# FabianPlum/SMILify

Measured on AMD Instinct MI355X. Metric: SMIL fit-iters/sec (LBS+render+loss) per GPU at 1/2/4/8 MI355X, higher is better.
Workload: dtype f32

## Files before the change

smilify_amd/csrc/raster.hip:

```cpp
#include "common.h"

#include "raster_hooks.h"
#include "raster_common.h"
#include "raster_setup.h"
#include "raster_tile.h"
#include "raster_replay.h"

static int device_cus() { return smil_device_limits().cus; }

static long long tile_slots() {
    long long resident = (long long)device_cus() * RESIDENT_PER_CU;
    HOOK_RESIDENT(resident)
    return resident;
}
static int tile_grid(int N, int tiles_x) {
    const long long resident = tile_slots();
    const unsigned long long n_max = (unsigned long long)N * tiles_x * tiles_x;
    const unsigned int slots = (unsigned int)resident;
    unsigned int best = slots / 8u;
    const unsigned long long ends[4] = {slots * 5ull / 64ull, slots * 5ull / 16ull, slots * 5ull / 8ull, n_max};
    for (int k = 0; k < 4; ++k) {
        const unsigned long long n = ends[k] < n_max ? ends[k] : n_max;
        if (n == 0ull || n > 0x7FFFFFFull) { if (n) best = slots; continue; }
        const unsigned int w = deal_working((unsigned int)n, deal_split_log((unsigned int)n, slots), slots);
// ... 18 lines not shown
    a.fzr = q.fzr = w.take<float2>((size_t)N * FT);
    a.gbox = q.gbox = w.take<uint32_t>((size_t)N * (FT / WAVE));
    a.img_bound = q.img_bound = w.take<float>(N);
    a.loss_acc = q.loss_acc = w.take<unsigned long long>(N);
    a.list_cap = q.list_cap = list_cap_of(m, S);
    a.lists = q.lists = w.take<uint2>((size_t)N * q.list_cap);
    ClipTables &c = q.clip;
    c.xv = w.take<float>((size_t)N * CLIP_VX * 3);
    c.xg = w.take<float>((size_t)N * CLIP_VX * 2);
    c.xsrc = w.take<int2>((size_t)N * CLIP_VX);
    c.xcoef = w.take<float2>((size_t)N * CLIP_VX);
    c.xf = w.take<int>((size_t)N * CLIP_FX * 3);
    c.xcount = w.take<uint32_t>(N);
    c.xparent = nullptr;
    a.clip = c;
    w.take<char>(256);
    const size_t grid = (size_t)tile_grid(N, tiles_x);
    a.list_stride = (int)(align256((size_t)FT * sizeof(uint32_t)) / sizeof(uint32_t));
    a.n_cf = (int)(align256((size_t)(FT / DCHUNK + 2) * sizeof(uint32_t)) / sizeof(uint32_t));
    a.slist = w.take<uint2>(grid * a.list_stride);
    a.slist2 = w.take<uint32_t>(grid * a.list_stride);
    a.scfirst = w.take<uint32_t>(grid * a.n_cf);
    a.sxy = w.take<float2>(grid * a.list_stride * 3);
    a.sid = w.take<TriIds>(grid * a.list_stride);
    a.srec = w.take<Rec3>(grid * (REC_CAP + REC_PAD));
    a.crec = w.take<Rec3>(grid * (REC_CAP + REC_PAD));
    return w.used;
}

extern "C" size_t smil_raster_workspace_bytes(const SmilModel *m, int32_t N, int32_t S) {
    SetupArgs q;
    RasterArgs a;
    return (m && N > 0 && S > 0) ? raster_layout(m, N, S, nullptr, q, a) : 0;
}

extern "C" int smil_raster_stats(const SmilModel *m, const void *workspace, void *stream_, uint32_t *out4) {
    SMIL_REQUIRE(m && workspace && out4, "smil_raster_stats: bad argument");
    RasterCounters h;
    SMIL_HIP(hipMemcpyAsync(&h, workspace, sizeof(h), hipMemcpyDeviceToHost, (hipStream_t)stream_));
    SMIL_HIP(hipStreamSynchronize((hipStream_t)stream_));
    unsigned int tiles = 0;
    for (int q = 0; q < N_PARTS; ++q)
        for (int c = 0; c < N_CLASSES; ++c) tiles += h.n_class[q][c];
    out4[0] = h.straddling; out4[1] = tiles; out4[2] = h.unclipped; out4[3] = h.tie_pixels;
    return SMIL_OK;
}

static int check_sizes(const SmilModel *m, int N, int S, const char *who) {
    SMIL_REQUIRE(N > 0 && S > 0 && S <= TILE * 256, "%s: bad sizes N=%d S=%d", who, N, S);
    const int tiles_x = ceil_div(S, TILE);
    SMIL_REQUIRE((double)N * tiles_x * tiles_x < 2147483647.0, "%s: N * tiles exceeds the work-item index range (2^31); launch in slices", who);
    SMIL_REQUIRE(face_rows(m) + 64 < (1 << 24) && (double)list_cap_of(m, S) * sizeof(uint2) < 4294967296.0,
                 "%s: per-workgroup / per-image tables exceed the 24-bit index / 32-bit byte-offset range of at()", who);
    return SMIL_OK;
}

static int launch_setup(SetupArgs &q, int N, hipStream_t stream) {
    SMIL_HIP(hipMemsetAsync(q.ctr, 0, sizeof(RasterCounters), stream));
    const int n_tiles = q.tiles_x * q.tiles_x;
    q.copies = n_tiles * 2 * 12 <= 48 * 1024 ? 2 : 1;
#ifdef SETUP_COPIES
    q.copies = SETUP_COPIES;
#endif
    const size_t setup_lds = n_tiles <= COUNT_TILES_MAX ? (size_t)n_tiles * q.copies * 12 : (size_t)((n_tiles + 31) / 32) * sizeof(uint32_t);
    hipLaunchKernelGGL(k_raster_setup, dim3(N), dim3(SETUP_THREADS), setup_lds, stream, q);
    SMIL_LAUNCH_CHECK();
    return SMIL_OK;
}

static int raster_common(const SmilModel *m, const float *verts_ndc, int N, int S, const SmilRasterSettings *rs, void *workspace,
                         hipStream_t stream, bool grads, SetupArgs &q, RasterArgs &a) {
    SMIL_REQUIRE(m && verts_ndc && rs && workspace, "raster: null argument");
    if (int rc = check_sizes(m, N, S, "raster")) return rc;
    SMIL_REQUIRE(rs->faces_per_pixel > 0 && rs->faces_per_pixel <= SMIL_MAX_FACES_PER_PIXEL,
                 "raster: faces_per_pixel=%d outside 1..%d", rs->faces_per_pixel, SMIL_MAX_FACES_PER_PIXEL);
    SMIL_REQUIRE(rs->sigma > 0.f && rs->blur_radius >= 0.f, "raster: bad blend settings");
    SMIL_REQUIRE(rs->tie_rule == SMIL_TIE_DEPTH_FACE_ID || rs->tie_rule == SMIL_TIE_REFERENCE_QUEUE, "raster: tie_rule=%d is neither 0 nor 1", rs->tie_rule);
    SMIL_REQUIRE(face_rows(m) <= REC_CAP, "raster: %d faces exceed the %d a single pixel's records may hold", m->F, REC_CAP - CLIP_FX - WAVE);
    static_assert(REC_CAP + REC_PAD < (1 << 24), "at<12-byte>() multiplies 24-bit indices");
    if (grads && rs->clip_depth)
        SMIL_REQUIRE(rs->clip_depth->vertex && rs->clip_depth->dz && rs->clip_depth->range && rs->clip_depth->counter && rs->clip_depth->capacity >= 0 &&
                     rs->image0 >= 0, "raster: incomplete SmilClipDepth");
    raster_layout(m, N, S, (char *)workspace, q, a);
    const int tiles_x = ceil_div(S, TILE);
    if (rs->tie_rule) SMIL_HIP(hipMemsetAsync(a.tie_mask, 0, (size_t)2 * N_PARTS * a.item_cap * sizeof(unsigned long long), stream));
    q.verts_ndc = a.verts_ndc = verts_ndc; q.faces = a.faces = m->faces;
    q.V = a.V = m->V; q.F = a.F = m->F; q.S = a.S = S; q.tiles_x = a.tiles_x = tiles_x;
    q.sqrt_blur = a.sqrt_blur = sqrtf(rs->blur_radius); q.z_clip = rs->z_clip; q.max_valence = m->max_valence;
    q.inv_sigma = a.inv_sigma = 1.0f / rs->sigma;
    q.cd_counter = (grads && rs->clip_depth && rs->image0 == 0) ? rs->clip_depth->counter : nullptr;
    if (int rc = launch_setup(q, N, stream)) return rc;
    a.FT = face_rows(m); a.slots = (unsigned int)tile_slots();
    a.tie_rule = rs->tie_rule; a.image0 = rs->image0;
    a.cd = (grads && rs->clip_depth) ? *rs->clip_depth : SmilClipDepth{nullptr, nullptr, nullptr, nullptr, 0};
    a.N = N; a.K = rs->faces_per_pixel; a.packed = 0;
    a.blur = rs->blur_radius; a.inv_sigma_log2e = (float)(1.4426950408889634 / (double)rs->sigma);
    HOOK_HOST_LAUNCH_SETUP(a, stream)
    a.sil = nullptr; a.grad_sil = nullptr; a.target = nullptr; a.target_u8 = nullptr; a.pix_scale = nullptr; a.loss_img = nullptr;
    a.d_ndc = nullptr;
    return SMIL_OK;
}

static size_t colour_setup_layout(const SmilModel *m, int N, int S, char *base, ColourSetup *o, SetupArgs *q) {
    const int tiles_x = ceil_div(S, TILE), FT = face_rows(m);
    const uint32_t item_cap = (uint32_t)ceil_div(N, N_PARTS) * (uint32_t)(tiles_x * tiles_x);
    const uint32_t list_cap = list_cap_of(m, S);
    Workspace w{base};
    uint32_t *tbox = w.take<uint32_t>((size_t)N * FT);
    RasterCounters *c = w.take<RasterCounters>(1);
    uint4 *items = w.take<uint4>((size_t)2 * N_PARTS * item_cap);
    float2 *fzr = w.take<float2>((size_t)N * FT);
    uint32_t *gbox = w.take<uint32_t>((size_t)N * (FT / WAVE));
    uint2 *lists = w.take<uint2>((size_t)N * list_cap);
    ClipTables clip;
    clip.xv = w.take<float>((size_t)N * CLIP_VX * 3);
    clip.xsrc = w.take<int2>((size_t)N * CLIP_VX);
    clip.xcoef = w.take<float2>((size_t)N * CLIP_VX);
    clip.xf = w.take<int>((size_t)N * CLIP_FX * 3);
    clip.xparent = w.take<int>((size_t)N * CLIP_CUTS);
    clip.xg = nullptr; clip.xcount = nullptr;
    if (!base) return w.used;
    o->tbox = tbox; o->gbox = gbox; o->fzr = fzr; o->items = items;
    o->n_class = &c->n_class[0][0]; o->ticket = &c->deal[0].next; o->item_cap = item_cap;
    o->lists = lists; o->list_cap = list_cap;
    o->xv = clip.xv; o->xf = clip.xf; o->xsrc = clip.xsrc; o->xparent = clip.xparent;
    o->FT = FT; o->FP = faces_padded(m->F); o->clip_vx = CLIP_VX; o->clip_fx = CLIP_FX; o->n_parts = N_PARTS; o->n_classes = N_CLASSES;
    *q = SetupArgs{};
    q->clip = clip; q->faces = m->faces; q->tbox = tbox; q->gbox = gbox; q->items = items;
    q->item_cap = item_cap; q->fzr = fzr; q->ctr = c; q->V = m->V; q->F = m->F; q->S = S; q->tiles_x = tiles_x;
    q->sqrt_blur = 0.f; q->inv_sigma = 1.f; q->lists = lists; q->list_cap = list_cap;
    return w.used;
}

size_t smil_colour_setup_bytes(const SmilModel *m, int N, int S) {
    return (m && N > 0 && S > 0) ? colour_setup_layout(m, N, S, nullptr, nullptr, nullptr) : 0;
}

int smil_colour_setup(const SmilModel *m, const float *verts_ndc, int N, int S, float z_clip, void *workspace, hipStream_t stream,
                      ColourSetup *out) {
    if (int rc = check_sizes(m, N, S, "smil_render_colour")) return rc;
    SetupArgs q;
    colour_setup_layout(m, N, S, (char *)workspace, out, &q);
    q.verts_ndc = verts_ndc; q.z_clip = z_clip;
    return launch_setup(q, N, stream);
}

#define PROF_SLOTS 512
static bool g_prof_on = false;
static hipEvent_t g_prof_ev[PROF_SLOTS][2];
static int g_prof_n = 0;
static bool g_prof_init = false;

extern "C" int smil_profile_enable(int32_t on) {
    if (on && !g_prof_init) {
        for (int i = 0; i < PROF_SLOTS; ++i) {
            SMIL_HIP(hipEventCreate(&g_prof_ev[i][0]));
            SMIL_HIP(hipEventCreate(&g_prof_ev[i][1]));
        }
        g_prof_init = true;
    }
    g_prof_on = on != 0;
    g_prof_n = 0;
    return SMIL_OK;
}

extern "C" int smil_profile_read(float *total_ms, int32_t *launches) {
    SMIL_REQUIRE(total_ms && launches, "smil_profile_read: null argument");
    float tot = 0.f;
    const int n = g_prof_n < PROF_SLOTS ? g_prof_n : PROF_SLOTS;
    for (int i = 0; i < n; ++i) {
        SMIL_HIP(hipEventSynchronize(g_prof_ev[i][1]));
        float ms = 0.f;
        SMIL_HIP(hipEventElapsedTime(&ms, g_prof_ev[i][0], g_prof_ev[i][1]));
        tot += ms;
    }
    *total_ms = tot;
    *launches = n;
    g_prof_n = 0;
    return SMIL_OK;
}

#define PROF_BEGIN(stream) \
    const int _slot = (g_prof_on && g_prof_n < PROF_SLOTS) ? g_prof_n++ : -1; \
    if (_slot >= 0) (void)hipEventRecord(g_prof_ev[_slot][0], stream)
#define PROF_END(stream) \
    if (_slot >= 0) (void)hipEventRecord(g_prof_ev[_slot][1], stream)

template <int MODE>
static void launch_tie_replay(const RasterArgs &a, hipStream_t stream) {
    const size_t lds = (size_t)a.FT / 8 + 6 * WAVE * sizeof(uint32_t) + (size_t)TIE_ORD_CAP * sizeof(uint16_t) + TIE_ORD_CAP / 8;
    if (a.tie_rule) hipLaunchKernelGGL((k_raster_tie_replay<MODE>), dim3((unsigned int)device_cus() * 4u * TIE_WAVES_PER_SIMD), dim3(64), lds, stream, a);
}
template <int MODE>
static int launch_raster(const RasterArgs &a, hipStream_t stream) {
    PROF_BEGIN(stream);
    hipLaunchKernelGGL((k_raster_dense<MODE>), dim3(tile_grid(a.N, a.tiles_x)), dim3(64), 0, stream, a);
    PROF_END(stream);
    launch_tie_replay<MODE>(a, stream);
    SMIL_LAUNCH_CHECK();
    return SMIL_OK;
}

extern "C" int smil_silhouette_forward(const SmilModel *m, const float *verts_ndc, int32_t N, int32_t S,
                                       const SmilRasterSettings *rs, float *sil, void *workspace, void *stream_) {
    hipStream_t stream = (hipStream_t)stream_;
    SetupArgs q{};
    RasterArgs a;
    int rc = raster_common(m, verts_ndc, N, S, rs, workspace, stream, false, q, a);
    if (rc) return rc;
    SMIL_REQUIRE(sil, "smil_silhouette_forward: null output");
    SMIL_HIP(hipMemsetAsync(sil, 0, (size_t)N * S * S * sizeof(float), stream));
    a.sil = sil;
    return launch_raster<MODE_FWD>(a, stream);
// ... 45 lines not shown
```

smilify_amd/csrc/raster_common.h:

```cpp
#pragma once

#define DCHUNK 32
#define FREC 28
#define FSTR 28
#define K_EPS 1e-8f
#define ALPHA_GRAD_EPS 1e-12f
#ifndef SEL_BITS
#define SEL_BITS 5
#endif
#ifndef SEL1_BITS
#define SEL1_BITS 6
#endif
#define SAT8 160u
#ifndef DGROUP
#define DGROUP 4
#endif
#ifndef KGROUP
#define KGROUP 4
#endif
#ifndef SELR
#define SELR 6
#endif
#ifndef LIST_LDS_ROWS
#define LIST_LDS_ROWS 8
// ... 68 lines not shown
struct RasterArgs {
    const float *verts_ndc;
    const int *faces;
    const uint32_t *tbox;
    const uint32_t *gbox;
    const uint4 *items;
    uint32_t item_cap;
    const float2 *fzr;
    RasterCounters *ctr;
    int N, V, F, S, tiles_x, K;
    int FT;
    ClipTables clip;
    float blur, sqrt_blur, inv_sigma, inv_sigma_log2e;
    float *sil;
    const float *grad_sil;
    const float *target;
    const uint8_t *target_u8;
    const float *pix_scale;
    const float *img_bound;
    int packed;
    float *loss_img;
    unsigned long long *loss_acc;
    float *d_ndc;
    const uint2 *lists;
    uint32_t list_cap;
    uint2 *slist;
    uint32_t *slist2;
    uint32_t *scfirst;
    float2 *sxy;
    TriIds *sid;
    Rec3 *srec;
    Rec3 *crec;
    int list_stride, n_cf;
    unsigned int slots;
    SmilClipDepth cd;
    int image0;
    int tie_rule;
    unsigned long long *tie_mask;
    HOOK_ARGS_FIELDS
};

__device__ __forceinline__ float tile_centre(int t, int S) { return pix_to_ndc(S - 1 - (t * TILE + TILE / 2), S); }

__device__ __forceinline__ float edge_fn(float px, float py, float ax, float ay, float bx, float by) {
    return (px - ax) * (by - ay) - (py - ay) * (bx - ax);
}

__device__ __forceinline__ float image_fx_scale(float img_bound, float pix_scale, float inv_sigma) {
    const float bound = img_bound * fabsf(pix_scale) * sqrtf(inv_sigma);
    return (bound > 0.f && bound < 3.0e38f) ? exp2f(fminf(29.0f - floorf(log2f(bound)), 100.0f)) : 0.f;
}

template <typename T>
__device__ __forceinline__ uint32_t byte_offset(uint32_t i) {
    if (sizeof(T) == 12) {
        uint32_t r;
        asm("v_mul_u32_u24 %0, %1, 12" : "=v"(r) : "v"(i));
        return r;
    }
    return i * (uint32_t)sizeof(T);
}
template <typename T>
__device__ __forceinline__ T &at(T *base, uint32_t i) {
    i = HOOK_WRAP_IDX(i);
    return *reinterpret_cast<T *>(reinterpret_cast<char *>(base) + byte_offset<T>(i));
}
template <typename T>
__device__ __forceinline__ const T &at(const T *base, uint32_t i) {
    i = HOOK_WRAP_IDX(i);
    return *reinterpret_cast<const T *>(reinterpret_cast<const char *>(base) + byte_offset<T>(i));
}

__device__ __forceinline__ int wave_scan_add(int x) {
#define SCAN_STEP(ctrl, rows) { x += __builtin_amdgcn_update_dpp(0, x, ctrl, rows, 0xF, false); }
    SCAN_STEP(0x111, 0xF) SCAN_STEP(0x112, 0xF) SCAN_STEP(0x114, 0xF) SCAN_STEP(0x118, 0xF)
    SCAN_STEP(0x142, 0xA) SCAN_STEP(0x143, 0xC)
#undef SCAN_STEP
    return x;
}

#ifndef SETUP_THREADS
#define SETUP_THREADS 1024
#endif
#ifndef LIST_CAP_PER_FACE
#define LIST_CAP_PER_FACE 8
#endif
struct SetupArgs {
    ClipTables clip;
    const float *verts_ndc; const int *faces;
    uint32_t *tbox, *gbox; uint4 *items; uint32_t item_cap; float2 *fzr;
    RasterCounters *ctr;
    int V, F, S, tiles_x; float sqrt_blur, z_clip;
    float *d_ndc_zero; const float *loss_src; float *loss_dst; unsigned long long *loss_acc; float *img_bound; int max_valence;
    float *dndc_scale; const float *pix_scale; float inv_sigma; int packed;
    uint2 *lists;
    uint32_t list_cap;
    uint32_t *cd_counter;
    int copies;
};

struct alignas(16) FaceRec {
    float A0, A1, B0, B1;
    float C0, C1, A2, B2;
    float C2, z0, z1, z2;
    float x0c, x1c, y0c, y1c;
    float e01x, e02x, e01y, e02y;
    float rl01, rl02, e12x, e12y;
    float rl12;
    int i0, i1, i2;
};
static_assert(sizeof(FaceRec) == FREC * sizeof(float), "FaceRec layout");

typedef float f32x2 __attribute__((ext_vector_type(2)));
__device__ __forceinline__ f32x2 splat2(float x) { return (f32x2){x, x}; }
__device__ __forceinline__ f32x2 clamp01(f32x2 v) {
    return __builtin_elementwise_min(__builtin_elementwise_max(v, splat2(0.f)), splat2(1.f));
}
__device__ __forceinline__ float vmax_raw(float a, float b) {
    float r;
    asm("v_max_f32 %0, %1, %2" : "=v"(r) : "v"(a), "v"(b));
    return r;
}

struct FaceRows { float4 r0, r1, r2, r3, r4, r5, r6; };
struct PairEval2 {
    f32x2 w0, w1, w2;
    f32x2 sd;
    bool cand0, cand1, inside0, inside1;
    uint32_t ebits0, ebits1;
};
__device__ __forceinline__ f32x2 pk_fma(f32x2 a, f32x2 b, f32x2 c) { return __builtin_elementwise_fma(a, b, c); }
__device__ __forceinline__ f32x2 pk_mul_clamp_lo(f32x2 v, f32x2 s2) {
    f32x2 r;
    asm("v_pk_mul_f32 %0, %1, %2 op_sel_hi:[1,0] clamp" : "=v"(r) : "v"(v), "v"(s2));
    return r;
}
__device__ __forceinline__ f32x2 pk_mul_clamp_hi(f32x2 v, f32x2 s2) {
    f32x2 r;
    asm("v_pk_mul_f32 %0, %1, %2 op_sel:[0,1] op_sel_hi:[1,1] clamp" : "=v"(r) : "v"(v), "v"(s2));
    return r;
}
__device__ __forceinline__ void eval_pair2(const FaceRows &q, float dx0, float dx1, float dyp, float blur, PairEval2 &e) {
    const f32x2 DX = {dx0, dx1};
    const f32x2 base01 = pk_fma((f32x2){q.r0.z, q.r0.w}, splat2(dyp), (f32x2){q.r1.x, q.r1.y});
    const float base2 = fmaf(q.r1.w, dyp, q.r2.x);
    e.w0 = pk_fma(splat2(q.r0.x), DX, splat2(base01.x));
    e.w1 = pk_fma(splat2(q.r0.y), DX, splat2(base01.y));
    e.w2 = pk_fma(splat2(q.r1.z), DX, splat2(base2));
    e.inside0 = fminf(fminf(e.w0.x, e.w1.x), e.w2.x) > 0.f;
    e.inside1 = fminf(fminf(e.w0.y, e.w1.y), e.w2.y) > 0.f;
    const f32x2 QX0 = DX - splat2(q.r3.x), QX1 = DX - splat2(q.r3.y);
    const f32x2 qy = splat2(dyp) - (f32x2){q.r3.z, q.r3.w};
    const f32x2 eyq0 = (f32x2){q.r4.z, q.r4.w} * splat2(qy.x);
    const float eyq12 = q.r5.w * qy.y;
    const f32x2 rl0102 = {q.r5.x, q.r5.y}, rl12_ = {q.r6.x, q.r6.y};
    const f32x2 T01 = pk_mul_clamp_lo(pk_fma(splat2(q.r4.x), QX0, splat2(eyq0.x)), rl0102);
    const f32x2 T02 = pk_mul_clamp_hi(pk_fma(splat2(q.r4.y), QX0, splat2(eyq0.y)), rl0102);
    const f32x2 T12 = pk_mul_clamp_lo(pk_fma(splat2(q.r5.z), QX1, splat2(eyq12)), rl12_);
    const f32x2 RX01 = pk_fma(T01, splat2(q.r4.x), -QX0), RY01 = pk_fma(T01, splat2(q.r4.z), -splat2(qy.x));
    const f32x2 RX02 = pk_fma(T02, splat2(q.r4.y), -QX0), RY02 = pk_fma(T02, splat2(q.r4.w), -splat2(qy.x));
    const f32x2 RX12 = pk_fma(T12, splat2(q.r5.z), -QX1), RY12 = pk_fma(T12, splat2(q.r5.w), -splat2(qy.y));
    const f32x2 D01 = pk_fma(RX01, RX01, RY01 * RY01), D02 = pk_fma(RX02, RX02, RY02 * RY02), D12 = pk_fma(RX12, RX12, RY12 * RY12);
    const float dist0 = fminf(fminf(D01.x, D02.x), D12.x), dist1 = fminf(fminf(D01.y, D02.y), D12.y);
    e.cand0 = e.inside0 || dist0 < blur;
    e.cand1 = e.inside1 || dist1 < blur;
    e.sd = (f32x2){e.inside0 ? -dist0 : dist0, e.inside1 ? -dist1 : dist1};
    e.ebits0 = D01.x == dist0 ? 0u : (D02.x == dist0 ? 1u << 23 : 2u << 23);
    e.ebits1 = D01.y == dist1 ? 0u : (D02.y == dist1 ? 1u << 23 : 2u << 23);
}
__device__ __forceinline__ f32x2 pair_depth2(const FaceRows &q, const PairEval2 &e) {
    float z0 = q.r2.y, z1 = q.r2.z, z2 = q.r2.w;
    asm("" : "+v"(z0), "+v"(z1), "+v"(z2));
    const f32x2 den3 = e.w0 + e.w1 + e.w2;
    const f32x2 den = {fmaxf(den3.x, K_EPS), fmaxf(den3.y, K_EPS)};
    const f32x2 m0 = {vmax_raw(e.w0.x, 0.f), vmax_raw(e.w0.y, 0.f)}, m1 = {vmax_raw(e.w1.x, 0.f), vmax_raw(e.w1.y, 0.f)},
                m2 = {vmax_raw(e.w2.x, 0.f), vmax_raw(e.w2.y, 0.f)};
    const f32x2 msum = m0 + m1 + m2, floor_ = splat2(1e-5f) * den;
    const f32x2 cs = {fmaxf(msum.x, floor_.x), fmaxf(msum.y, floor_.y)};
    const f32x2 rc = {__builtin_amdgcn_rcpf(cs.x), __builtin_amdgcn_rcpf(cs.y)};
    const f32x2 pz = pk_fma(splat2(z2), m2 * rc, pk_fma(splat2(z0), m0 * rc, splat2(z1) * (m1 * rc)));
// ... 78 lines not shown
```

smilify_amd/csrc/raster_setup.h:

```cpp
#pragma once

__global__ void __launch_bounds__(SETUP_THREADS, 8) k_raster_setup(SetupArgs q) {
    __shared__ uint32_t s_maxpx;
    __shared__ uint32_t s_straddle;
    __shared__ uint32_t s_zext;
    if (threadIdx.x == 0) { s_maxpx = 0u; s_straddle = 0u; s_zext = 0u; }
    uint32_t my_px = 0u, my_straddle = 0u;
    float my_zext = 0.f;
    extern __shared__ __align__(16) unsigned long long tcnt64[];
    TSETUP_INIT
    const int n = blockIdx.x;
    const int V = q.V, F = q.F, S = q.S, tiles_x = q.tiles_x;
    if (q.d_ndc_zero) {
        float2 *z = reinterpret_cast<float2 *>(q.d_ndc_zero) + (size_t)n * V;
        for (int i = threadIdx.x; i < V; i += blockDim.x) z[i] = make_float2(0.f, 0.f);
    }
    if (q.loss_dst && threadIdx.x == 0) { q.loss_dst[n] = q.loss_src[n]; q.loss_acc[n] = 0ull; }
    if (q.cd_counter && n == 0 && threadIdx.x == 0) { q.cd_counter[0] = 0u; q.cd_counter[1] = 0u; }
    const int n_tiles = tiles_x * tiles_x;
    const bool counted = n_tiles <= COUNT_TILES_MAX;
    uint32_t *const tbits = reinterpret_cast<uint32_t *>(tcnt64);
    const int KC = counted ? q.copies : 1;
    uint32_t *const tcur = reinterpret_cast<uint32_t *>(tcnt64 + KC * n_tiles);
    if (counted) { for (int i = threadIdx.x; i < KC * n_tiles; i += blockDim.x) tcnt64[i] = 0ull; }
    else { for (int i = threadIdx.x; i < (n_tiles + 31) >> 5; i += blockDim.x) tbits[i] = 0u; }
    __syncthreads();
    const float *vn = q.verts_ndc + (size_t)n * V * 3;
    const float fS = (float)S;
    const int FP = faces_padded(F), FT = FP + CLIP_FX;
    const int n_groups = FT / WAVE;
    __shared__ uint32_t s_ncut, s_unclipped;
    __shared__ int s_cut[CLIP_CUTS];
    if (threadIdx.x == 0) { s_ncut = 0u; s_unclipped = 0u; }
    for (int i = threadIdx.x; i < FT - F; i += blockDim.x) q.tbox[(size_t)n * FT + F + i] = 0x0000FFFFu;
    __syncthreads();
    TSETUP(1)
    float *const xv_n = q.clip.xv + (size_t)n * CLIP_VX * 3;
    int *const xf_n = q.clip.xf + (size_t)n * CLIP_FX * 3;
    auto emit = [&](int fid, float x0, float y0, float z0, float x1, float y1, float z1, float x2, float y2, float z2) -> uint32_t {
        uint32_t box = 0x0000FFFFu;
        const float zmin = fminf(fminf(z0, z1), z2), zmax = fmaxf(fmaxf(z0, z1), z2);
        const float area = edge_fn(x0, y0, x1, y1, x2, y2);
        const bool finite = (x0 == x0) && (x1 == x1) && (x2 == x2) && (y0 == y0) && (y1 == y1) && (y2 == y2);
        if (finite && !(zmin < K_EPS) && !(zmax < q.z_clip) && !(area <= K_EPS && area >= -K_EPS)) {
            const float xlo = fminf(fminf(x0, x1), x2) - q.sqrt_blur, xhi = fmaxf(fmaxf(x0, x1), x2) + q.sqrt_blur;
            const float ylo = fminf(fminf(y0, y1), y2) - q.sqrt_blur, yhi = fmaxf(fmaxf(y0, y1), y2) + q.sqrt_blur;
            const float vxl = fminf(fmaxf(((xlo + 1.0f) * fS - 1.0f) * 0.5f - 0.01f, -1.0f), fS), vxh = fminf(fmaxf(((xhi + 1.0f) * fS - 1.0f) * 0.5f + 0.01f, -1.0f), fS);
            const float vyl = fminf(fmaxf(((ylo + 1.0f) * fS - 1.0f) * 0.5f - 0.01f, -1.0f), fS), vyh = fminf(fmaxf(((yhi + 1.0f) * fS - 1.0f) * 0.5f + 0.01f, -1.0f), fS);
            int xi_lo = (int)ceilf(vxl), xi_hi = (int)floorf(vxh), yi_lo = (int)ceilf(vyl), yi_hi = (int)floorf(vyh);
            xi_lo = max(xi_lo, 0); yi_lo = max(yi_lo, 0);
            xi_hi = min(xi_hi, S - 1); yi_hi = min(yi_hi, S - 1);
            if (xi_lo <= xi_hi && yi_lo <= yi_hi) {
                my_px = max(my_px, (uint32_t)((xi_hi - xi_lo + 1) * (yi_hi - yi_lo + 1)));
                my_zext = fmaxf(my_zext, zmax - zmin);
                const int tx0 = (S - 1 - xi_hi) / TILE, tx1 = (S - 1 - xi_lo) / TILE;
                const int ty0 = (S - 1 - yi_hi) / TILE, ty1 = (S - 1 - yi_lo) / TILE;
                box = (uint32_t)tx0 | ((uint32_t)ty0 << 8) | ((uint32_t)tx1 << 16) | ((uint32_t)ty1 << 24);
                const int xo0 = S - 1 - xi_hi, xo1 = S - 1 - xi_lo, yo0 = S - 1 - yi_hi, yo1 = S - 1 - yi_lo;
                for (int ty = ty0; ty <= ty1; ++ty)
                    for (int tx = tx0; tx <= tx1; ++tx) {
                        const int t = ty * tiles_x + tx;
                        if (counted) {
                            const int wx = min(xo1, tx * TILE + TILE - 1) - max(xo0, tx * TILE) + 1;
                            const int wy = min(yo1, ty * TILE + TILE - 1) - max(yo0, ty * TILE) + 1;
                            HOOK_SETUP_COUNT(atomicAdd(&tcnt64[(fid & (KC - 1)) * n_tiles + t], (1ull << 32) | (unsigned long long)(uint32_t)(wx * wy + 8));)
                        } else {
                            atomicOr(&tbits[t >> 5], 1u << (t & 31));
                        }
                    }
            }
        }
        q.tbox[(size_t)n * FT + fid] = box;
        q.fzr[(size_t)n * FT + fid] = make_float2(zmin, zmax);
        return box;
    };
    int nx0 = 0, nx1 = 0, nx2 = 0;
    if ((int)threadIdx.x < F) { nx0 = q.faces[3 * threadIdx.x]; nx1 = q.faces[3 * threadIdx.x + 1]; nx2 = q.faces[3 * threadIdx.x + 2]; }
    for (int f0 = 0; f0 < FP; f0 += blockDim.x) {
        const int f = f0 + threadIdx.x;
        uint32_t box = 0x0000FFFFu;
        const int ii[3] = {nx0, nx1, nx2};
        {
            const int fn = min(f + (int)blockDim.x, F - 1);
            nx0 = q.faces[3 * fn]; nx1 = q.faces[3 * fn + 1]; nx2 = q.faces[3 * fn + 2];
        }
        if (f < F) {
            float X[3], Y[3], Z[3];
#pragma unroll
            for (int k = 0; k < 3; ++k) { X[k] = vn[3 * ii[k]]; Y[k] = vn[3 * ii[k] + 1]; Z[k] = vn[3 * ii[k] + 2]; }
            const int nb = (Z[0] < q.z_clip ? 1 : 0) + (Z[1] < q.z_clip ? 1 : 0) + (Z[2] < q.z_clip ? 1 : 0);
            const bool finite = (X[0] == X[0]) && (X[1] == X[1]) && (X[2] == X[2]) && (Y[0] == Y[0]) && (Y[1] == Y[1]) && (Y[2] == Y[2]) &&
                                (Z[0] == Z[0]) && (Z[1] == Z[1]) && (Z[2] == Z[2]);
            bool cut = false;
            if (finite && (nb == 1 || nb == 2)) {
                ++my_straddle;
                const uint32_t c = q.clip.xv ? atomicAdd(&s_ncut, 1u) : (uint32_t)CLIP_CUTS;
                if (c < (uint32_t)CLIP_CUTS) {
                    s_cut[c] = f;
                    cut = true;
                    q.tbox[(size_t)n * FT + f] = 0x0000FFFFu;
                    q.fzr[(size_t)n * FT + f] = make_float2(fminf(fminf(Z[0], Z[1]), Z[2]), fmaxf(fmaxf(Z[0], Z[1]), Z[2]));
                } else {
                    atomicAdd(&s_unclipped, 1u);
                }
            }
            if (!cut) box = emit(f, X[0], Y[0], Z[0], X[1], Y[1], Z[1], X[2], Y[2], Z[2]);
        }
        int gx0 = box & 0xFF, gy0 = (box >> 8) & 0xFF, gx1 = (box >> 16) & 0xFF, gy1 = box >> 24;
        for (int o = 32; o > 0; o >>= 1) {
            gx0 = min(gx0, __shfl_xor(gx0, o, WAVE)); gy0 = min(gy0, __shfl_xor(gy0, o, WAVE));
            gx1 = max(gx1, __shfl_xor(gx1, o, WAVE)); gy1 = max(gy1, __shfl_xor(gy1, o, WAVE));
        }
        const int grp = (f0 + (int)threadIdx.x) / WAVE;
        if ((threadIdx.x & (WAVE - 1)) == 0 && grp < FP / WAVE)
            q.gbox[(size_t)n * n_groups + grp] = (uint32_t)gx0 | ((uint32_t)gy0 << 8) | ((uint32_t)gx1 << 16) | ((uint32_t)gy1 << 24);
    }
    __syncthreads();
    TSETUP(2)
    const uint32_t n_cut = min(s_ncut, (uint32_t)CLIP_CUTS);
    for (uint32_t c = threadIdx.x; c < n_cut; c += blockDim.x) {
        const int f = s_cut[c];
        if (q.clip.xparent) q.clip.xparent[(size_t)n * CLIP_CUTS + c] = f;
        const int ii[3] = {q.faces[3 * f], q.faces[3 * f + 1], q.faces[3 * f + 2]};
        float X[3], Y[3], Z[3];
        for (int k = 0; k < 3; ++k) { X[k] = vn[3 * ii[k]]; Y[k] = vn[3 * ii[k] + 1]; Z[k] = vn[3 * ii[k] + 2]; }
        const int nb = (Z[0] < q.z_clip ? 1 : 0) + (Z[1] < q.z_clip ? 1 : 0) + (Z[2] < q.z_clip ? 1 : 0);
        const int k1 = nb == 1 ? (Z[0] < q.z_clip ? 0 : (Z[1] < q.z_clip ? 1 : 2)) : (!(Z[0] < q.z_clip) ? 0 : (!(Z[1] < q.z_clip) ? 1 : 2));
        const int o1 = k1, o2 = (k1 + 1) % 3, o3 = (k1 + 2) % 3;
        const uint32_t jv = 2u * c;
        float nx[2], ny[2];
        for (int e = 0; e < 2; ++e) {
            const int a = o1, b = e == 0 ? o2 : o3;
            const float wb = (Z[a] - q.z_clip) / (Z[a] - Z[b]);
            const float ca = Z[a] * (1.0f - wb) / q.z_clip, cb = Z[b] * wb / q.z_clip;
            nx[e] = ca * X[a] + cb * X[b]; ny[e] = ca * Y[a] + cb * Y[b];
            float *o = xv_n + 3 * (jv + e);
            o[0] = nx[e]; o[1] = ny[e]; o[2] = q.z_clip;
            q.clip.xsrc[(size_t)n * CLIP_VX + jv + e] = make_int2(ii[a], ii[b]);
            q.clip.xcoef[(size_t)n * CLIP_VX + jv + e] = make_float2(ca, cb);
        }
        const int v4 = V + (int)jv, v5 = v4 + 1;
        int *xf = xf_n + 3 * (2 * c);
        if (nb == 1) {
            xf[0] = v4; xf[1] = ii[o2]; xf[2] = ii[o3]; xf[3] = v4; xf[4] = ii[o3]; xf[5] = v5;
            emit(FP + 2 * (int)c, nx[0], ny[0], q.z_clip, X[o2], Y[o2], Z[o2], X[o3], Y[o3], Z[o3]);
            emit(FP + 2 * (int)c + 1, nx[0], ny[0], q.z_clip, X[o3], Y[o3], Z[o3], nx[1], ny[1], q.z_clip);
        } else {
            xf[0] = ii[o1]; xf[1] = v4; xf[2] = v5;
            emit(FP + 2 * (int)c, X[o1], Y[o1], Z[o1], nx[0], ny[0], q.z_clip, nx[1], ny[1], q.z_clip);
        }
    }
    __syncthreads();
    TSETUP(3)
    static_assert(CLIP_FX % WAVE == 0 && SETUP_THREADS % WAVE == 0, "whole waves of front-part faces");
    for (int i = threadIdx.x; i < CLIP_FX; i += blockDim.x) {
        const uint32_t box = i < 2 * (int)n_cut ? q.tbox[(size_t)n * FT + FP + i] : 0x0000FFFFu;
        int gx0 = box & 0xFF, gy0 = (box >> 8) & 0xFF, gx1 = (box >> 16) & 0xFF, gy1 = box >> 24;
        for (int o = 32; o > 0; o >>= 1) {
            gx0 = min(gx0, __shfl_xor(gx0, o, WAVE)); gy0 = min(gy0, __shfl_xor(gy0, o, WAVE));
            gx1 = max(gx1, __shfl_xor(gx1, o, WAVE)); gy1 = max(gy1, __shfl_xor(gy1, o, WAVE));
        }
        if ((i & (WAVE - 1)) == 0)
            q.gbox[(size_t)n * n_groups + FP / WAVE + i / WAVE] = (uint32_t)gx0 | ((uint32_t)gy0 << 8) | ((uint32_t)gx1 << 16) | ((uint32_t)gy1 << 24);
    }
    if (q.clip.xcount) {
        const uint32_t nxv = 2u * n_cut;
        if (threadIdx.x == 0) q.clip.xcount[n] = nxv;
        for (int i = threadIdx.x; i < (int)nxv * 2; i += blockDim.x) q.clip.xg[(size_t)n * CLIP_VX * 2 + i] = 0.f;
    }
    if (threadIdx.x == 0 && s_unclipped) atomicAdd(&q.ctr->unclipped, s_unclipped);
    {
        uint32_t zb = __float_as_uint(my_zext);
        for (int o = 32; o > 0; o >>= 1) {
            my_px = max(my_px, (uint32_t)__shfl_xor((int)my_px, o, WAVE));
            zb = max(zb, (uint32_t)__shfl_xor((int)zb, o, WAVE));
            my_straddle += (uint32_t)__shfl_xor((int)my_straddle, o, WAVE);
        }
        if ((threadIdx.x & (WAVE - 1)) == 0) {
            if (my_px) atomicMax(&s_maxpx, my_px);
            if (zb) atomicMax(&s_zext, zb);
            if (my_straddle) atomicAdd(&s_straddle, my_straddle);
        }
    }
    __syncthreads();
    TSETUP(4)
    if (threadIdx.x == 0 && q.img_bound) {
        const float bound = 1.02f * 0.4f * (float)q.max_valence * (float)s_maxpx;
        q.img_bound[n] = bound;
        if (q.dndc_scale) {
            const bool pk = q.packed && s_ncut == 0u;
            const float sc = pk ? image_fx_scale(bound, q.pix_scale[n], q.inv_sigma) : 0.f;
            q.dndc_scale[n] = sc > 0.f ? 1.0f / sc : (pk ? -1.0f : 0.f);
        }
    }
    if (threadIdx.x == 0 && s_straddle) atomicAdd(&q.ctr->straddling, s_straddle);
    __shared__ uint32_t s_cnt[N_CLASSES], s_base[N_CLASSES], s_ents[SETUP_THREADS / WAVE], s_binned;
    if (threadIdx.x < N_CLASSES) s_cnt[threadIdx.x] = 0u;
    __syncthreads();
    auto tile_class = [&](int t) -> int {
        if (!counted) return ((tbits[t >> 5] >> (t & 31)) & 1u) ? N_CLASSES - 1 : -1;
        uint32_t c = 0u;
        for (int k = 0; k < KC; ++k) c += (uint32_t)tcnt64[k * n_tiles + t];
        return c == 0u ? -1 : (c >= CLASS_T0 ? 0 : (c >= CLASS_T1 ? 1 : (c >= CLASS_T2 ? 2 : 3)));
    };
    uint32_t mine[N_CLASSES] = {0u, 0u, 0u, 0u};
    uint32_t my_ents = 0u;
    for (int t = threadIdx.x; t < n_tiles; t += blockDim.x) {
        const int c = tile_class(t);
#pragma unroll
        for (int k = 0; k < N_CLASSES; ++k) mine[k] += (c == k) ? 1u : 0u;
        if (counted)
            for (int k = 0; k < KC; ++k) my_ents += (uint32_t)(tcnt64[k * n_tiles + t] >> 32);
    }
    uint32_t off[N_CLASSES];
#pragma unroll
    for (int k = 0; k < N_CLASSES; ++k) off[k] = mine[k] ? atomicAdd(&s_cnt[k], mine[k]) : 0u;
    const uint32_t incl = (uint32_t)wave_scan_add((int)my_ents);
    if ((threadIdx.x & (WAVE - 1)) == WAVE - 1) s_ents[threadIdx.x / WAVE] = incl;
    __syncthreads();
    TSETUP(5)
    uint32_t ent_off = incl - my_ents;
    for (int w = 0; w < (int)(threadIdx.x / WAVE); ++w) ent_off += s_ents[w];
    if (threadIdx.x == blockDim.x - 1) s_binned = (counted && q.list_cap != 0u && ent_off + my_ents <= q.list_cap) ? 1u : 0u;
    const int part = n % N_PARTS;
    if (threadIdx.x < N_CLASSES) s_base[threadIdx.x] = s_cnt[threadIdx.x] ? atomicAdd(&q.ctr->n_class[part][threadIdx.x], s_cnt[threadIdx.x]) : 0u;
    __syncthreads();
    TSETUP(6)
    const bool binned = s_binned != 0u;
#pragma unroll
    for (int k = 0; k < N_CLASSES; ++k) off[k] += s_base[k];
    uint32_t run = ent_off;
    const uint32_t zext_bits = s_zext;
    for (int t = threadIdx.x; t < n_tiles; t += blockDim.x) {
        const int c = tile_class(t);
        uint32_t e = 0u;
        const uint32_t first = run;
        if (counted)
            for (int k = 0; k < KC; ++k) {
                if (binned) tcur[k * n_tiles + t] = run + e;
                e += (uint32_t)(tcnt64[k * n_tiles + t] >> 32);
            }
        run += e;
        if (c < 0) continue;
        uint32_t slot = 0u;
#pragma unroll
        for (int k = 0; k < N_CLASSES; ++k)
            if (c == k) slot = off[k]++;
        const uint32_t idx = (uint32_t)(2 * part + (c >> 1)) * q.item_cap + ((c & 1) ? q.item_cap - 1u - slot : slot);
        q.items[idx] = make_uint4((uint32_t)n * (uint32_t)n_tiles + (uint32_t)t, binned ? first : 0u, binned ? e : 0xFFFFFFFFu, zext_bits);
    }
    if (!binned) return;
    __syncthreads();
    TSETUP(7)
    uint2 *const lists = q.lists + (size_t)n * q.list_cap;
    const int f_end = FP + 2 * (int)n_cut;
    for (int f = threadIdx.x; f < f_end; f += blockDim.x) {
        const uint32_t box = q.tbox[(size_t)n * FT + f];
        const uint2 ent = make_uint2((uint32_t)f, __float_as_uint(q.fzr[(size_t)n * FT + f].x));
        const int tx0 = box & 0xFF, ty0 = (box >> 8) & 0xFF, tx1 = (box >> 16) & 0xFF, ty1 = box >> 24;
        if (tx0 > tx1) continue;
        uint32_t *const cur = tcur + (f & (KC - 1)) * n_tiles;
        for (int ty = ty0; ty <= ty1; ++ty)
            for (int tx = tx0; tx <= tx1; ++tx) at(lists, atomicAdd(&cur[ty * tiles_x + tx], 1u)) = ent;
    }
    TSETUP(8)
    TSETUP_REPORT
}

__global__ void __launch_bounds__(256) k_unpack_dndc(float *__restrict__ d_ndc, const float *__restrict__ img_bound,
                                                     const float *__restrict__ pix_scale, float inv_sigma, int V,
                                                     const uint32_t *__restrict__ xcount) {
    const int n = blockIdx.x, v = blockIdx.y * blockDim.x + threadIdx.x;
    if (v >= V || (xcount && xcount[n] != 0u)) return;
    const float sc = image_fx_scale(img_bound[n], pix_scale[n], inv_sigma);
    const float inv = sc > 0.f ? 1.0f / sc : 0.f;
    unsigned long long *p = reinterpret_cast<unsigned long long *>(d_ndc) + (size_t)n * V + v;
    const unsigned long long tot = *p;
    const int qy = (int)(uint32_t)tot;
    const int qx = (int)(uint32_t)((tot - (unsigned long long)(long long)qy) >> 32);
    *reinterpret_cast<float2 *>(p) = make_float2((float)qx * inv, (float)qy * inv);
}

__global__ void __launch_bounds__(64) k_clip_backward(ClipTables c, float *__restrict__ d_ndc, int V, float *__restrict__ loss_img,
                                                      const unsigned long long *__restrict__ loss_acc, const float *__restrict__ verts_ndc,
                                                      float z_clip, SmilClipDepth cd, int image0) {
    const int n = blockIdx.x;
    if (loss_img && threadIdx.x == 0) loss_img[n] += (float)((double)(long long)loss_acc[n] * (1.0 / 4294967296.0));
    const uint32_t nx = c.xcount[n];
    __shared__ uint32_t s_first;
    if (cd.range) {
        if (threadIdx.x == 0) {
            uint32_t first = 0u, cnt = 0u;
            if (nx) {
                first = atomicAdd(&cd.counter[0], 2u * nx);
                if (first + 2u * nx <= (uint32_t)cd.capacity) cnt = 2u * nx;
                else atomicAdd(&cd.counter[1], 2u * nx);
            }
            cd.range[2 * (size_t)(image0 + n)] = first;
            cd.range[2 * (size_t)(image0 + n) + 1] = cnt;
            s_first = cnt ? first : 0xFFFFFFFFu;
        }
        __syncthreads();
    }
    const uint32_t zfirst = cd.range ? s_first : 0xFFFFFFFFu;
    const float *vn = verts_ndc + (size_t)n * V * 3;
    for (uint32_t j = threadIdx.x; j < nx; j += blockDim.x) {
        const float gx = c.xg[((size_t)n * CLIP_VX + j) * 2], gy = c.xg[((size_t)n * CLIP_VX + j) * 2 + 1];
        const int2 ab = c.xsrc[(size_t)n * CLIP_VX + j];
        if (zfirst != 0xFFFFFFFFu) {
            const float xa = vn[3 * ab.x], ya = vn[3 * ab.x + 1], za = vn[3 * ab.x + 2];
            const float xb = vn[3 * ab.y], yb = vn[3 * ab.y + 1], zb = vn[3 * ab.y + 2];
            const float inv = 1.0f / (za - zb);
            const float ge = fmaf(gx, xb - xa, gy * (yb - ya)) * (inv * inv) * (1.0f / z_clip);
            cd.vertex[zfirst + 2u * j] = ab.x;
            cd.dz[zfirst + 2u * j] = ge * (zb * (z_clip - zb));
            cd.vertex[zfirst + 2u * j + 1u] = ab.y;
            cd.dz[zfirst + 2u * j + 1u] = ge * (za * (za - z_clip));
        }
        if (gx == 0.f && gy == 0.f) continue;
        const float2 co = c.xcoef[(size_t)n * CLIP_VX + j];
        float *da = d_ndc + ((size_t)n * V + ab.x) * 2, *db = d_ndc + ((size_t)n * V + ab.y) * 2;
        atomicAdd(da, co.x * gx); atomicAdd(da + 1, co.x * gy);
        atomicAdd(db, co.y * gx); atomicAdd(db + 1, co.y * gy);
    }
}
```

Baseline: 76.14.

## Keep per-face tile boxes and near depth in registers during raster setup

The setup kernel now holds each thread's face tile box and near-z in register arrays across up to SETUP_REG_ROUNDS rounds. When the tie rule is depth/face-id and binning lists exist, it skips writing tbox/fzr/gbox to global memory and bins faces straight from registers; in the unbinned path it writes the tables at the end. It also moves the per-wave max-px and z-extent reductions into the loop and counts straddling faces with a direct shared atomic. This cuts global stores and reloads but raises register pressure and adds branching complexity.

Result: faster. 77.45 (median of 6 runs) (+1.7%).

```diff
diff --git a/smilify_amd/csrc/raster.hip b/smilify_amd/csrc/raster.hip
--- a/smilify_amd/csrc/raster.hip
+++ b/smilify_amd/csrc/raster.hip
@@ -124,6 +124,7 @@
         SMIL_REQUIRE(rs->clip_depth->vertex && rs->clip_depth->dz && rs->clip_depth->range && rs->clip_depth->counter && rs->clip_depth->capacity >= 0 &&
                      rs->image0 >= 0, "raster: incomplete SmilClipDepth");
     raster_layout(m, N, S, (char *)workspace, q, a);
+    q.store_tables = (rs->tie_rule != SMIL_TIE_DEPTH_FACE_ID || q.list_cap == 0u) ? 1 : 0;
     const int tiles_x = ceil_div(S, TILE);
     if (rs->tie_rule) SMIL_HIP(hipMemsetAsync(a.tie_mask, 0, (size_t)2 * N_PARTS * a.item_cap * sizeof(unsigned long long), stream));
     q.verts_ndc = a.verts_ndc = verts_ndc; q.faces = a.faces = m->faces;
@@ -171,6 +172,7 @@
     q->clip = clip; q->faces = m->faces; q->tbox = tbox; q->gbox = gbox; q->items = items;
     q->item_cap = item_cap; q->fzr = fzr; q->ctr = c; q->V = m->V; q->F = m->F; q->S = S; q->tiles_x = tiles_x;
     q->sqrt_blur = 0.f; q->inv_sigma = 1.f; q->lists = lists; q->list_cap = list_cap;
+    q->store_tables = 1;
     return w.used;
 }
 
diff --git a/smilify_amd/csrc/raster_common.h b/smilify_amd/csrc/raster_common.h
--- a/smilify_amd/csrc/raster_common.h
+++ b/smilify_amd/csrc/raster_common.h
@@ -174,6 +174,9 @@
 #ifndef SETUP_THREADS
 #define SETUP_THREADS 1024
 #endif
+#ifndef SETUP_REG_ROUNDS
+#define SETUP_REG_ROUNDS 6
+#endif
 #ifndef LIST_CAP_PER_FACE
 #define LIST_CAP_PER_FACE 8
 #endif
@@ -188,6 +191,7 @@
     uint2 *lists;
     uint32_t list_cap;
     uint32_t *cd_counter;
+    int store_tables;
     int copies;
 };
 
diff --git a/smilify_amd/csrc/raster_setup.h b/smilify_amd/csrc/raster_setup.h
--- a/smilify_amd/csrc/raster_setup.h
+++ b/smilify_amd/csrc/raster_setup.h
@@ -5,7 +5,7 @@
     __shared__ uint32_t s_straddle;
     __shared__ uint32_t s_zext;
     if (threadIdx.x == 0) { s_maxpx = 0u; s_straddle = 0u; s_zext = 0u; }
-    uint32_t my_px = 0u, my_straddle = 0u;
+    uint32_t my_px = 0u;
     float my_zext = 0.f;
     extern __shared__ __align__(16) unsigned long long tcnt64[];
     TSETUP_INIT
@@ -32,14 +32,22 @@
     __shared__ uint32_t s_ncut, s_unclipped;
     __shared__ int s_cut[CLIP_CUTS];
     if (threadIdx.x == 0) { s_ncut = 0u; s_unclipped = 0u; }
-    for (int i = threadIdx.x; i < FT - F; i += blockDim.x) q.tbox[(size_t)n * FT + F + i] = 0x0000FFFFu;
+    const bool in_regs = FP <= SETUP_REG_ROUNDS * (int)blockDim.x;
+    const bool store = q.store_tables != 0 || !in_regs;
+    uint32_t rbox[SETUP_REG_ROUNDS], rzn[SETUP_REG_ROUNDS];
+#pragma unroll
+    for (int r = 0; r < SETUP_REG_ROUNDS; ++r) { rbox[r] = 0x0000FFFFu; rzn[r] = 0u; }
+    if (store)
+        for (int i = threadIdx.x; i < FT - F; i += blockDim.x) q.tbox[(size_t)n * FT + F + i] = 0x0000FFFFu;
     __syncthreads();
     TSETUP(1)
     float *const xv_n = q.clip.xv + (size_t)n * CLIP_VX * 3;
     int *const xf_n = q.clip.xf + (size_t)n * CLIP_FX * 3;
-    auto emit = [&](int fid, float x0, float y0, float z0, float x1, float y1, float z1, float x2, float y2, float z2) -> uint32_t {
+    auto emit = [&](int fid, float x0, float y0, float z0, float x1, float y1, float z1, float x2, float y2, float z2, float &znear) -> uint32_t {
         uint32_t box = 0x0000FFFFu;
         const float zmin = fminf(fminf(z0, z1), z2), zmax = fmaxf(fmaxf(z0, z1), z2);
+        znear = zmin;
+        if (store || fid >= FP) q.fzr[(size_t)n * FT + fid] = make_float2(zmin, zmax);
         const float area = edge_fn(x0, y0, x1, y1, x2, y2);
         const bool finite = (x0 == x0) && (x1 == x1) && (x2 == x2) && (y0 == y0) && (y1 == y1) && (y2 == y2);
         if (finite && !(zmin < K_EPS) && !(zmax < q.z_clip) && !(area <= K_EPS && area >= -K_EPS)) {
@@ -51,11 +59,11 @@
             xi_lo = max(xi_lo, 0); yi_lo = max(yi_lo, 0);
             xi_hi = min(xi_hi, S - 1); yi_hi = min(yi_hi, S - 1);
             if (xi_lo <= xi_hi && yi_lo <= yi_hi) {
-                my_px = max(my_px, (uint32_t)((xi_hi - xi_lo + 1) * (yi_hi - yi_lo + 1)));
                 my_zext = fmaxf(my_zext, zmax - zmin);
                 const int tx0 = (S - 1 - xi_hi) / TILE, tx1 = (S - 1 - xi_lo) / TILE;
                 const int ty0 = (S - 1 - yi_hi) / TILE, ty1 = (S - 1 - yi_lo) / TILE;
                 box = (uint32_t)tx0 | ((uint32_t)ty0 << 8) | ((uint32_t)tx1 << 16) | ((uint32_t)ty1 << 24);
+                if (store || fid >= FP) q.tbox[(size_t)n * FT + fid] = box;
                 const int xo0 = S - 1 - xi_hi, xo1 = S - 1 - xi_lo, yo0 = S - 1 - yi_hi, yo1 = S - 1 - yi_lo;
                 for (int ty = ty0; ty <= ty1; ++ty)
                     for (int tx = tx0; tx <= tx1; ++tx) {
@@ -68,17 +76,28 @@
                             atomicOr(&tbits[t >> 5], 1u << (t & 31));
                         }
                     }
-            }
-        }
-        q.tbox[(size_t)n * FT + fid] = box;
-        q.fzr[(size_t)n * FT + fid] = make_float2(zmin, zmax);
+                my_px = max(my_px, (uint32_t)((xo1 - xo0 + 1) * (yo1 - yo0 + 1)));
+            }
+        }
+        if ((store || fid >= FP) && box == 0x0000FFFFu) q.tbox[(size_t)n * FT + fid] = box;
         return box;
     };
+    auto wave_box = [&](uint32_t box) -> uint32_t {
+        const uint32_t gx0 = 255u - wave_max_u32(255u - (box & 0xFFu)), gy0 = 255u - wave_max_u32(255u - ((box >> 8) & 0xFFu));
+        const uint32_t gx1 = wave_max_u32((box >> 16) & 0xFFu), gy1 = wave_max_u32(box >> 24);
+        return gx0 | (gy0 << 8) | (gx1 << 16) | (gy1 << 24);
+    };
+    auto group_box = [&](uint32_t box, int grp) {
+        const uint32_t g = wave_box(box);
+        if ((threadIdx.x & (WAVE - 1)) == 0 && grp < FP / WAVE) q.gbox[(size_t)n * n_groups + grp] = g;
+    };
     int nx0 = 0, nx1 = 0, nx2 = 0;
+    uint32_t wave_px = 0u, wave_zext = 0u;
     if ((int)threadIdx.x < F) { nx0 = q.faces[3 * threadIdx.x]; nx1 = q.faces[3 * threadIdx.x + 1]; nx2 = q.faces[3 * threadIdx.x + 2]; }
     for (int f0 = 0; f0 < FP; f0 += blockDim.x) {
         const int f = f0 + threadIdx.x;
         uint32_t box = 0x0000FFFFu;
+        float znear = 0.f;
         const int ii[3] = {nx0, nx1, nx2};
         {
             const int fn = min(f + (int)blockDim.x, F - 1);
@@ -93,28 +112,37 @@
                                 (Z[0] == Z[0]) && (Z[1] == Z[1]) && (Z[2] == Z[2]);
             bool cut = false;
             if (finite && (nb == 1 || nb == 2)) {
-                ++my_straddle;
+                atomicAdd(&s_straddle, 1u);
                 const uint32_t c = q.clip.xv ? atomicAdd(&s_ncut, 1u) : (uint32_t)CLIP_CUTS;
                 if (c < (uint32_t)CLIP_CUTS) {
                     s_cut[c] = f;
                     cut = true;
-                    q.tbox[(size_t)n * FT + f] = 0x0000FFFFu;
-                    q.fzr[(size_t)n * FT + f] = make_float2(fminf(fminf(Z[0], Z[1]), Z[2]), fmaxf(fmaxf(Z[0], Z[1]), Z[2]));
+                    if (store) {
+                        q.tbox[(size_t)n * FT + f] = 0x0000FFFFu;
+                        q.fzr[(size_t)n * FT + f] = make_float2(fminf(fminf(Z[0], Z[1]), Z[2]), fmaxf(fmaxf(Z[0], Z[1]), Z[2]));
+                    }
                 } else {
                     atomicAdd(&s_unclipped, 1u);
                 }
             }
-            if (!cut) box = emit(f, X[0], Y[0], Z[0], X[1], Y[1], Z[1], X[2], Y[2], Z[2]);
-        }
-        int gx0 = box & 0xFF, gy0 = (box >> 8) & 0xFF, gx1 = (box >> 16) & 0xFF, gy1 = box >> 24;
-        for (int o = 32; o > 0; o >>= 1) {
-            gx0 = min(gx0, __shfl_xor(gx0, o, WAVE)); gy0 = min(gy0, __shfl_xor(gy0, o, WAVE));
-            gx1 = max(gx1, __shfl_xor(gx1, o, WAVE)); gy1 = max(gy1, __shfl_xor(gy1, o, WAVE));
-        }
-        const int grp = (f0 + (int)threadIdx.x) / WAVE;
-        if ((threadIdx.x & (WAVE - 1)) == 0 && grp < FP / WAVE)
-            q.gbox[(size_t)n * n_groups + grp] = (uint32_t)gx0 | ((uint32_t)gy0 << 8) | ((uint32_t)gx1 << 16) | ((uint32_t)gy1 << 24);
-    }
+            if (!cut) box = emit(f, X[0], Y[0], Z[0], X[1], Y[1], Z[1], X[2], Y[2], Z[2], znear);
+        }
+        if (in_regs) {
+#pragma unroll
+            for (int r = 0; r < SETUP_REG_ROUNDS; ++r) {
+                const bool here = f0 == r * (int)blockDim.x;
+                rbox[r] = here ? box : rbox[r];
+                rzn[r] = here ? __float_as_uint(znear) : rzn[r];
+            }
+        }
+        if (store) group_box(box, (f0 + (int)threadIdx.x) / WAVE);
+        wave_px = max(wave_px, wave_max_u32(my_px));
+        wave_zext = max(wave_zext, wave_max_u32(__float_as_uint(my_zext)));
+        my_px = 0u;
+        my_zext = 0.f;
+    }
+    my_px = wave_px;
+    my_zext = __uint_as_float(wave_zext);
     __syncthreads();
     TSETUP(2)
     const uint32_t n_cut = min(s_ncut, (uint32_t)CLIP_CUTS);
@@ -128,7 +156,13 @@
         const int k1 = nb == 1 ? (Z[0] < q.z_clip ? 0 : (Z[1] < q.z_clip ? 1 : 2)) : (!(Z[0] < q.z_clip) ? 0 : (!(Z[1] < q.z_clip) ? 1 : 2));
         const int o1 = k1, o2 = (k1 + 1) % 3, o3 = (k1 + 2) % 3;
         const uint32_t jv = 2u * c;
-        float nx[2], ny[2];
+        float nx[2], ny[2], zn_;
+        {
+            const int v4 = V + (int)jv, v5 = v4 + 1;
+            int *xf = xf_n + 3 * (2 * c);
+            if (nb == 1) { xf[0] = v4; xf[1] = ii[o2]; xf[2] = ii[o3]; xf[3] = v4; xf[4] = ii[o3]; xf[5] = v5; }
+            else { xf[0] = ii[o1]; xf[1] = v4; xf[2] = v5; }
+        }
         for (int e = 0; e < 2; ++e) {
             const int a = o1, b = e == 0 ? o2 : o3;
             const float wb = (Z[a] - q.z_clip) / (Z[a] - Z[b]);
@@ -139,30 +173,25 @@
             q.clip.xsrc[(size_t)n * CLIP_VX + jv + e] = make_int2(ii[a], ii[b]);
             q.clip.xcoef[(size_t)n * CLIP_VX + jv + e] = make_float2(ca, cb);
         }
-        const int v4 = V + (int)jv, v5 = v4 + 1;
-        int *xf = xf_n + 3 * (2 * c);
         if (nb == 1) {
-            xf[0] = v4; xf[1] = ii[o2]; xf[2] = ii[o3]; xf[3] = v4; xf[4] = ii[o3]; xf[5] = v5;
-            emit(FP + 2 * (int)c, nx[0], ny[0], q.z_clip, X[o2], Y[o2], Z[o2], X[o3], Y[o3], Z[o3]);
-            emit(FP + 2 * (int)c + 1, nx[0], ny[0], q.z_clip, X[o3], Y[o3], Z[o3], nx[1], ny[1], q.z_clip);
+            emit(FP + 2 * (int)c, nx[0], ny[0], q.z_clip, X[o2], Y[o2], Z[o2], X[o3], Y[o3], Z[o3], zn_);
+            emit(FP + 2 * (int)c + 1, nx[0], ny[0], q.z_clip, X[o3], Y[o3], Z[o3], nx[1], ny[1], q.z_clip, zn_);
         } else {
-            xf[0] = ii[o1]; xf[1] = v4; xf[2] = v5;
-            emit(FP + 2 * (int)c, X[o1], Y[o1], Z[o1], nx[0], ny[0], q.z_clip, nx[1], ny[1], q.z_clip);
+            emit(FP + 2 * (int)c, X[o1], Y[o1], Z[o1], nx[0], ny[0], q.z_clip, nx[1], ny[1], q.z_clip, zn_);
+            q.tbox[(size_t)n * FT + FP + 2 * (int)c + 1] = 0x0000FFFFu;
         }
     }
     __syncthreads();
     TSETUP(3)
     static_assert(CLIP_FX % WAVE == 0 && SETUP_THREADS % WAVE == 0, "whole waves of front-part faces");
-    for (int i = threadIdx.x; i < CLIP_FX; i += blockDim.x) {
-        const uint32_t box = i < 2 * (int)n_cut ? q.tbox[(size_t)n * FT + FP + i] : 0x0000FFFFu;
-        int gx0 = box & 0xFF, gy0 = (box >> 8) & 0xFF, gx1 = (box >> 16) & 0xFF, gy1 = box >> 24;
-        for (int o = 32; o > 0; o >>= 1) {
-            gx0 = min(gx0, __shfl_xor(gx0, o, WAVE)); gy0 = min(gy0, __shfl_xor(gy0, o, WAVE));
-            gx1 = max(gx1, __shfl_xor(gx1, o, WAVE)); gy1 = max(gy1, __shfl_xor(gy1, o, WAVE));
-        }
-        if ((i & (WAVE - 1)) == 0)
-            q.gbox[(size_t)n * n_groups + FP / WAVE + i / WAVE] = (uint32_t)gx0 | ((uint32_t)gy0 << 8) | ((uint32_t)gx1 << 16) | ((uint32_t)gy1 << 24);
-    }
+    auto front_group_boxes = [&]() {
+        for (int i = threadIdx.x; i < CLIP_FX; i += blockDim.x) {
+            const uint32_t box = i < 2 * (int)n_cut ? q.tbox[(size_t)n * FT + FP + i] : 0x0000FFFFu;
+            const uint32_t g = wave_box(box);
+            if ((i & (WAVE - 1)) == 0) q.gbox[(size_t)n * n_groups + FP / WAVE + i / WAVE] = g;
+        }
+    };
+    if (store) front_group_boxes();
     if (q.clip.xcount) {
         const uint32_t nxv = 2u * n_cut;
         if (threadIdx.x == 0) q.clip.xcount[n] = nxv;
@@ -174,12 +203,10 @@
         for (int o = 32; o > 0; o >>= 1) {
             my_px = max(my_px, (uint32_t)__shfl_xor((int)my_px, o, WAVE));
             zb = max(zb, (uint32_t)__shfl_xor((int)zb, o, WAVE));
-            my_straddle += (uint32_t)__shfl_xor((int)my_straddle, o, WAVE);
         }
         if ((threadIdx.x & (WAVE - 1)) == 0) {
             if (my_px) atomicMax(&s_maxpx, my_px);
             if (zb) atomicMax(&s_zext, zb);
-            if (my_straddle) atomicAdd(&s_straddle, my_straddle);
         }
     }
     __syncthreads();
@@ -249,20 +276,44 @@
         const uint32_t idx = (uint32_t)(2 * part + (c >> 1)) * q.item_cap + ((c & 1) ? q.item_cap - 1u - slot : slot);
         q.items[idx] = make_uint4((uint32_t)n * (uint32_t)n_tiles + (uint32_t)t, binned ? first : 0u, binned ? e : 0xFFFFFFFFu, zext_bits);
     }
-    if (!binned) return;
+    if (!binned) {
+        if (!store) {
+            for (int i = threadIdx.x + 2 * (int)n_cut; i < CLIP_FX; i += blockDim.x) q.tbox[(size_t)n * FT + FP + i] = 0x0000FFFFu;
+#pragma unroll
+            for (int r = 0; r < SETUP_REG_ROUNDS; ++r) {
+                const int f = r * (int)blockDim.x + (int)threadIdx.x;
+                if (r * (int)blockDim.x < FP) {
+                    if (f < FP) q.tbox[(size_t)n * FT + f] = rbox[r];
+                    if (f < F) {
+                        const float z0 = vn[3 * q.faces[3 * f] + 2], z1 = vn[3 * q.faces[3 * f + 1] + 2], z2 = vn[3 * q.faces[3 * f + 2] + 2];
+                        q.fzr[(size_t)n * FT + f] = make_float2(fminf(fminf(z0, z1), z2), fmaxf(fmaxf(z0, z1), z2));
+                    }
+                    group_box(rbox[r], f / WAVE);
+                }
+            }
+            front_group_boxes();
+        }
+        return;
+    }
     __syncthreads();
     TSETUP(7)
     uint2 *const lists = q.lists + (size_t)n * q.list_cap;
     const int f_end = FP + 2 * (int)n_cut;
-    for (int f = threadIdx.x; f < f_end; f += blockDim.x) {
-        const uint32_t box = q.tbox[(size_t)n * FT + f];
-        const uint2 ent = make_uint2((uint32_t)f, __float_as_uint(q.fzr[(size_t)n * FT + f].x));
+    auto bin_face = [&](int f, uint32_t box, uint32_t znear_bits) {
+        const uint2 ent = make_uint2((uint32_t)f, znear_bits);
         const int tx0 = box & 0xFF, ty0 = (box >> 8) & 0xFF, tx1 = (box >> 16) & 0xFF, ty1 = box >> 24;
-        if (tx0 > tx1) continue;
+        if (tx0 > tx1) return;
         uint32_t *const cur = tcur + (f & (KC - 1)) * n_tiles;
         for (int ty = ty0; ty <= ty1; ++ty)
             for (int tx = tx0; tx <= tx1; ++tx) at(lists, atomicAdd(&cur[ty * tiles_x + tx], 1u)) = ent;
-    }
+    };
+    if (in_regs) {
+#pragma unroll
+        for (int r = 0; r < SETUP_REG_ROUNDS; ++r)
+            if (r * (int)blockDim.x < FP) bin_face(r * (int)blockDim.x + (int)threadIdx.x, rbox[r], rzn[r]);
+    }
+    for (int f = (in_regs ? FP : 0) + (int)threadIdx.x; f < f_end; f += blockDim.x)
+        bin_face(f, q.tbox[(size_t)n * FT + f], __float_as_uint(q.fzr[(size_t)n * FT + f].x));
     TSETUP(8)
     TSETUP_REPORT
 }
```
